# AnnaUshnova/tinyrenderder

Hardware: AMD Instinct MI355X
Metric: triangles/sec (+ Mpixels/sec) at 4096x4096; achieved HBM GB/s vs peak (higher is better)
Workload: dtype f64

## Files before the change

### profiles/binning_bytes.py

```python
import argparse
import csv
import glob
import re
from collections import defaultdict

BIN = ("k_chunk_spine", "k_expand", "k_radix_hist", "k_radix_scan_rows", "k_radix_scatter", "k_bounds", "k_make_items")


def short(name):
    m = re.search(r"k_radix_scatter<(?:\d+, )?(true|false), (true|false)>", name)
    if m:
        return "k_radix_scatter" + (" (last pass)" if m.group(2) == "true" else "")
    for k in BIN + ("k_setup", "k_raster", "k_fold_stats"):
        if k in name:
            return k
    return name.split("(")[0][:38]


ap = argparse.ArgumentParser()
ap.add_argument("--trace")
ap.add_argument("--pmc", nargs="*", default=[])
ap.add_argument("--pairs", type=int, required=True)
ap.add_argument("--tris", type=int, required=True)
ap.add_argument("--old", action="store_true")
a = ap.parse_args()
P, N = a.pairs, a.tris


def binning(name):
    return name.split(" ")[0] in BIN


if a.trace:
    acc = defaultdict(list)
    for f in glob.glob(f"{a.trace}/**/*kernel_trace.csv", recursive=True):
        for r in csv.DictReader(open(f)):
            acc[short(r["Kernel_Name"])].append((int(r["End_Timestamp"]) - int(r["Start_Timestamp"])) / 1e3)
    frames = len(acc["k_setup"])
    print(f"== kernel trace: {frames} frames ==")
    tot = 0.0
    for n, v in sorted(acc.items(), key=lambda kv: -sum(kv[1])):
        tot += sum(v) / frames if binning(n) else 0.0
        print(f"  {n:38s} calls {len(v):4d}  avg {sum(v) / len(v):8.1f} us  median {sorted(v)[len(v) // 2]:8.1f} us  per frame {sum(v) / frames:8.1f} us")
    print(f"  binning kernels per frame: {tot:.1f} us\n")

if a.pmc:
    cnt = defaultdict(lambda: defaultdict(list))
    for d in a.pmc:
        for f in glob.glob(f"{d}/**/*counter_collection.csv", recursive=True):
            per = defaultdict(float)
            for r in csv.DictReader(open(f)):
                n = short(r["Kernel_Name"])
                if binning(n):
                    per[(n, r["Dispatch_Id"], r["Counter_Name"])] += float(r["Counter_Value"])
            for (n, disp, c), v in per.items():
                cnt[n][c].append(v)
    per_frame = {"k_radix_hist": 2, "k_radix_scan_rows": 2, "k_radix_scatter": 2 if a.old else 1}
    if a.old:
        model = {"k_expand": (12 * N, 8 * P), "k_radix_hist": (2 * P, 0), "k_radix_scatter": (8 * P, 8 * P), "k_bounds": (2 * P, 0)}
    else:
        model = {"k_expand": (12 * N, 8 * P), "k_radix_hist": (4 * P, 0), "k_radix_scatter": (8 * P, 8 * P),
                 "k_radix_scatter (last pass)": (8 * P, 6 * P)}
    print("== PMC per dispatch (means) ==")
    for n in sorted(cnt):
        cs = cnt[n]
        print(f"  {n:30s} " + "  ".join(f"{c}={sum(v) / len(v):.4g}" for c, v in sorted(cs.items())))
        act, conf = sum(cs.get("SQ_LDS_IDX_ACTIVE", [0])), sum(cs.get("SQ_LDS_BANK_CONFLICT", [0]))
        if act:
            print(f"  {'':30s} SQ_LDS_BANK_CONFLICT / SQ_LDS_IDX_ACTIVE = {conf / act:.3f}")
    print(f"\n== bytes per frame (P = {P} pairs, N = {N} triangles; MB = 1e6 B) ==")
    print(f"  {'kernel':30s} {'x':>2s} {'read':>8s} {'model':>8s} {'write':>8s} {'model':>8s}")
    tr = tw = mr = mw = 0.0
    for n in sorted(cnt):
        cs = cnt[n]
        if "FETCH_SIZE" not in cs or "WRITE_SIZE" not in cs:
            continue
        k = per_frame.get(n, 1)
        r = 2 * 1024 * sum(cs["FETCH_SIZE"]) / len(cs["FETCH_SIZE"]) * k
        w = 1024 * sum(cs["WRITE_SIZE"]) / len(cs["WRITE_SIZE"]) * k
        m_r, m_w = (x * k for x in model.get(n, (0, 0)))
        tr += r; tw += w; mr += m_r; mw += m_w
        print(f"  {n:30s} {k:2d} {r / 1e6:8.1f} {m_r / 1e6:8.1f} {w / 1e6:8.1f} {m_w / 1e6:8.1f}"
              + (f"   read {100 * (r / m_r - 1):+.0f} %" if m_r else "") + (f", write {100 * (w / m_w - 1):+.0f} %" if m_w else ""))
    print(f"  {'total':30s}    {tr / 1e6:8.1f} {mr / 1e6:8.1f} {tw / 1e6:8.1f} {mw / 1e6:8.1f}")
    print(f"  measured {(tr + tw) / 1e6:.1f} MB against the model's {(mr + mw) / 1e6:.1f} MB: {100 * ((tr + tw) / (mr + mw) - 1):+.1f} %")
```

### tinyrenderder_amd/api.py

```python
from __future__ import annotations

import ctypes as C
import os
import sys

import numpy as np

HERE = os.path.dirname(os.path.abspath(__file__))
LIB_PATH = os.path.join(HERE, "libtrgl.so")

FLAT, GOURAUD, PHONG, EYE, CHECKER = 0, 1, 2, 3, 4
VARY = {FLAT: 0, GOURAUD: 3, PHONG: 24, EYE: 24, CHECKER: 0}
SHADER_USER_FIRST, MAX_USER_SHADERS, MAX_USER_VARY = 64, 32, 64
SHADER_MAY_DISCARD = 1
MAX_USER_VERTEX_SHADERS = 32
MEM_HOST, MEM_DEVICE = 0, 1
PHASE_SETUP, PHASE_BIN, PHASE_RASTER, PHASE_TOTAL, PHASE_RASTER_KERNEL = 0, 1, 2, 3, 4
NUM_PHASES = 5
MAX_TEXTURES = 16
MAX_Z_SNAPSHOTS = 4
MAX_BLUR_RADIUS = 46340
FRUSTUM_LEFT, FRUSTUM_RIGHT, FRUSTUM_BOTTOM, FRUSTUM_TOP, FRUSTUM_NEAR, FRUSTUM_FAR = range(6)

SYMBOLS = [
# ... 31 lines not shown
        return (self.triangles_rasterized, self.fragments_drawn, self.min_x, self.min_y, self.max_x, self.max_y,
                self.min_z, self.max_z, math.copysign(1.0, self.min_z), math.copysign(1.0, self.max_z))


class SsaoParams(C.Structure):
    _fields_ = [("num_directions", C.c_int32), ("steps_per_direction", C.c_int32), ("sample_radius", C.c_double),
                ("occlusion_threshold", C.c_double), ("intensity", C.c_double)]


def make_uniforms(model_view=None, key=(0, 0, 1), fill=(0, 0, 1), rim=(0, 0, 1), normal_map_strength=1.0,
                  tex_diffuse=-1, tex_normal=-1, tex_specular=-1, cells=0) -> Uniforms:
    u = Uniforms()
    mv = np.eye(4) if model_view is None else np.asarray(model_view, np.float64)
    u.model_view[:] = mv.reshape(16).tolist()
    u.key_light_dir_eye[:] = list(map(float, key))
    u.fill_light_dir_eye[:] = list(map(float, fill))
    u.rim_light_dir_eye[:] = list(map(float, rim))
    u.normal_map_strength = float(normal_map_strength)
    u.tex_diffuse, u.tex_normal, u.tex_specular, u.reserved = tex_diffuse, tex_normal, tex_specular, int(cells)
    return u


class TrglError(RuntimeError):
    pass


TRI_REC = np.dtype([(n, "<f8") for n in ("ax", "ay", "s0x", "s0y", "s1x", "s1y", "c0", "uz", "g1", "g2", "ruz", "z0", "z1", "z2")]
                   + [(n, "<u2") for n in ("bx0", "by0", "bx1", "by1")] + [("color", "<u4"), ("dl", "<u4")])
assert TRI_REC.itemsize == 128, "TRI_REC must mirror sizeof(TriRec) == 128"
DBG_RECS, DBG_CNT, DBG_TILEBOX, DBG_VALS, DBG_BMASK, DBG_TILE_START, DBG_TILE_END, DBG_INFO = range(8)
DBG_INFO_FIELDS = ("N", "P", "capacity", "wide", "literal_tris", "large_tris", "zq_cull", "pending", "W", "H", "tiles_x", "tiles_y",
                   "strip_y0", "strip_y1", "strip_ty0", "strip_ty1", "il_tiles", "il_world", "il_rank", "side")
DL_LITERAL = 0x80000000


_lib = None


def load_library(path: str = None):
    global _lib
    if _lib is not None:
        return _lib
    path = path or os.environ.get("TRGL_LIB") or LIB_PATH
    if "torch" not in sys.modules and not os.environ.get("TRGL_NO_TORCH_PRELOAD"):
        try:
            import torch
        except ImportError:
            pass
    if not os.path.exists(path):
        raise TrglError(f"{path} not found: build it with `python -c 'import __graft_entry__ as g; g.build()'` "
                        "(hipcc --offload-arch=gfx950). There is no CPU fallback.")
    L = C.CDLL(path)
    vp, u64p, dp = C.c_void_p, C.POINTER(C.c_uint64), C.POINTER(C.c_double)
    L.trgl_create.argtypes = [C.c_int, C.c_int, C.c_int, C.c_int, C.POINTER(vp)]
    L.trgl_destroy.argtypes = [vp]
    L.trgl_last_error.argtypes = [vp]; L.trgl_last_error.restype = C.c_char_p
    L.trgl_set_viewport.argtypes = [vp, dp]
    L.trgl_init_viewport.argtypes = [vp, C.c_int, C.c_int, C.c_int, C.c_int]
    L.trgl_clear.argtypes = [vp, C.c_void_p, C.c_double]
    L.trgl_upload_texture.argtypes = [vp, C.c_int, C.c_void_p, C.c_int, C.c_int, C.c_int]
    L.trgl_set_strip.argtypes = [vp, C.c_int, C.c_int]
    L.trgl_set_interleave.argtypes = [vp, C.c_int, C.c_int, C.c_int]
    L.trgl_draw.argtypes = [vp, C.c_int, C.POINTER(Uniforms), C.c_void_p, C.c_void_p, C.c_void_p, C.c_uint64, C.c_int]
    L.trgl_flush.argtypes = [vp]
    L.trgl_flush_begin.argtypes = [vp]
    L.trgl_flush_end.argtypes = [vp]
    L.trgl_sync.argtypes = [vp]
    L.trgl_read_framebuffer.argtypes = [vp, C.c_void_p]
    L.trgl_write_framebuffer.argtypes = [vp, C.c_void_p]
    L.trgl_read_zbuffer.argtypes = [vp, C.c_void_p]
    L.trgl_write_zbuffer.argtypes = [vp, C.c_void_p]
    L.trgl_get_stats.argtypes = [vp, C.POINTER(Stats)]
    L.trgl_reset_stats.argtypes = [vp]
    L.trgl_format_stats.argtypes = [C.POINTER(Stats), C.c_char_p, C.c_size_t]
    for name in ("trgl_framebuffer_device_ptr", "trgl_zbuffer_device_ptr", "trgl_stream"):
        getattr(L, name).argtypes = [vp]; getattr(L, name).restype = C.c_void_p
    L.trgl_set_stream.argtypes = [vp, C.c_void_p, C.c_int]
    L.trgl_set_profiling.argtypes = [vp, C.c_int]
    L.trgl_get_phase_ms.argtypes = [vp, dp, u64p]
    L.trgl_reset_phase_ms.argtypes = [vp]
    L.trgl_get_last_flush_info.argtypes = [vp, u64p, u64p, u64p]
    if hasattr(L, "trgl_debug_read"):
        L.trgl_debug_read.argtypes = [vp, C.c_int, C.c_void_p, C.c_size_t, C.POINTER(C.c_size_t)]
    L.trgl_selftest_division.argtypes = [vp, C.c_uint64, C.c_uint64, u64p]
    L.trgl_selftest_sampler.argtypes = [vp, C.c_int, C.c_void_p, C.c_uint64, C.c_void_p]
    L.trgl_draw_indexed.argtypes = [vp, C.c_int, C.POINTER(Uniforms), dp, C.c_void_p, C.c_int, C.c_uint64, C.c_void_p, C.c_uint64, C.c_int]
    L.trgl_ssao_defaults.argtypes = [C.POINTER(SsaoParams)]
    L.trgl_ssao_defaults.restype = None
    L.trgl_postprocess.argtypes = [vp, C.POINTER(SsaoParams), C.c_void_p, C.c_void_p, C.c_void_p]
    L.trgl_obj_load.argtypes = [C.c_char_p, C.POINTER(C.POINTER(C.c_double)), u64p, C.POINTER(C.POINTER(C.c_uint32)), u64p]
    L.trgl_obj_free.argtypes = [C.POINTER(C.c_double), C.POINTER(C.c_uint32)]
    L.trgl_obj_free.restype = None
    L.trgl_tga_max_size.argtypes = [C.c_int, C.c_int, C.c_int]
    L.trgl_tga_max_size.restype = C.c_size_t
    L.trgl_tga_encode.argtypes = [C.c_void_p, C.c_int, C.c_int, C.c_int, C.c_int, C.c_int, C.c_void_p, C.POINTER(C.c_size_t)]
    L.trgl_tga_info.argtypes = [C.c_void_p, C.c_size_t, C.POINTER(C.c_int), C.POINTER(C.c_int), C.POINTER(C.c_int)]
    L.trgl_tga_decode.argtypes = [C.c_void_p, C.c_size_t, C.c_void_p]
    L.trgl_gather.argtypes = [vp, C.c_void_p, C.c_int, C.c_int, C.c_int]
    L.trgl_rccl_unique_id.argtypes = [C.c_void_p]
    L.trgl_rccl_comm_create.argtypes = [C.c_void_p, C.c_int, C.c_int, C.c_int, C.POINTER(C.c_void_p)]
    L.trgl_rccl_comm_destroy.argtypes = [C.c_void_p]
    L.trgl_shader_compile.argtypes = [C.c_char_p, C.c_int, C.c_char_p, C.c_size_t]
    L.trgl_register_shader.argtypes = [vp, C.c_char_p, C.c_int, C.POINTER(C.c_int)]
    L.trgl_shader_compile_ex.argtypes = [C.c_char_p, C.c_int, C.c_uint32, C.c_char_p, C.c_size_t]
    L.trgl_register_shader_ex.argtypes = [vp, C.c_char_p, C.c_int, C.c_uint32, C.POINTER(C.c_int)]
    L.trgl_vertex_shader_compile.argtypes = [C.c_char_p, C.c_int, C.c_char_p, C.c_size_t]
    L.trgl_register_vertex_shader.argtypes = [vp, C.c_char_p, C.c_int, C.POINTER(C.c_int)]
    L.trgl_draw_indexed_vs.argtypes = [vp, C.c_int, C.c_int, C.POINTER(Uniforms), dp, C.c_void_p, C.c_int, C.c_uint64, C.c_void_p, C.c_uint64,
                                       C.c_void_p, C.c_int]
    L.trgl_vertex_stage.argtypes = [vp, C.c_int, C.POINTER(Uniforms), dp, C.c_void_p, C.c_int, C.c_uint64, C.c_void_p, C.c_uint64,
                                    C.c_void_p, C.c_void_p, C.c_int]
    L.trgl_mesh_bounds.argtypes = [vp, C.c_void_p, C.c_int, C.c_uint64, C.c_int, dp, dp]
    for name in ("trgl_mesh_normals", "trgl_mesh_tangents"):
        getattr(L, name).argtypes = [vp, C.c_void_p, C.c_int, C.c_uint64, C.c_void_p, C.c_uint64, C.c_int, C.POINTER(C.c_int)]
    L.trgl_aabb_transform.argtypes = [dp, dp, dp, dp, dp]
    L.trgl_frustum_from_matrix.argtypes = [dp, dp]
    L.trgl_frustum_intersects.argtypes = [dp, dp, dp]
    for name in ("trgl_zbuffer_snapshot", "trgl_zbuffer_restore", "trgl_zbuffer_snapshot_free"):
        getattr(L, name).argtypes = [vp, C.c_int]
    L.trgl_gaussian_kernel.argtypes = [C.c_int, C.c_void_p]
    L.trgl_image_blur.argtypes = [vp, C.c_void_p, C.c_int, C.c_int, C.c_int, C.c_int, C.c_int]
    L.trgl_image_scale.argtypes = [vp, C.c_void_p, C.c_int, C.c_int, C.c_int, C.c_void_p, C.c_int, C.c_int, C.c_int]
    L.trgl_framebuffer_blur.argtypes = [vp, C.c_int]
    for name in SYMBOLS:
        f = getattr(L, name)
        if f.restype is C.c_int and name not in ("trgl_last_error",):
            f.restype = C.c_int
    _lib = L
    return L


def rccl_unique_id() -> bytes:
    L = load_library()
    buf = (C.c_uint8 * 128)()
    rc = L.trgl_rccl_unique_id(buf)
    if rc != 0:
        raise TrglError(f"trgl_rccl_unique_id failed ({rc}): {L.trgl_last_error(None).decode()}")
    return bytes(buf)


def rccl_comm_create(unique_id: bytes, rank: int, world: int, device: int = 0):
    L = load_library()
    comm = C.c_void_p()
    buf = (C.c_uint8 * 128).from_buffer_copy(unique_id)
    rc = L.trgl_rccl_comm_create(buf, rank, world, device, C.byref(comm))
    if rc != 0:
        raise TrglError(f"trgl_rccl_comm_create failed ({rc}): {L.trgl_last_error(None).decode()}")
    return comm


def rccl_comm_destroy(comm):
    load_library().trgl_rccl_comm_destroy(comm)


def shader_compile(source: str, n_varyings: int, may_discard: bool = False):
    L = load_library()
    log = C.create_string_buffer(16384)
    rc = L.trgl_shader_compile_ex(source.encode(), int(n_varyings), SHADER_MAY_DISCARD if may_discard else 0, log, len(log))
    if rc not in (0, -1):
        raise TrglError(f"trgl_shader_compile failed ({rc}): {log.value.decode(errors='replace')}")
    return rc == 0, log.value.decode(errors="replace")


def vertex_shader_compile(source: str, n_varyings: int):
    L = load_library()
    log = C.create_string_buffer(16384)
# ... 526 lines not shown
```

### tinyrenderder_amd/csrc/kernels_bin.hip

```cpp
#include <hip/hip_runtime.h>
#include "trgl_device.h"
#include "launch.h"

namespace {

__device__ __forceinline__ double dmin3(double a, double b, double c) { double m = a; if (b < m) m = b; if (c < m) m = c; return m; }
__device__ __forceinline__ double dmax3(double a, double b, double c) { double m = a; if (m < b) m = b; if (m < c) m = c; return m; }
__device__ __forceinline__ double dot4(const double* m, const double* v) {
    double sum = 0;
    sum += m[0] * v[0]; sum += m[1] * v[1]; sum += m[2] * v[2]; sum += m[3] * v[3];
    return sum;
}

__device__ __forceinline__ int wave_min_i(int v) {
    for (int o = 32; o; o >>= 1) { int t = __shfl_xor(v, o); v = t < v ? t : v; }
    return v;
}
__device__ __forceinline__ int wave_max_i(int v) {
    for (int o = 32; o; o >>= 1) { int t = __shfl_xor(v, o); v = t > v ? t : v; }
    return v;
}

constexpr int SETUP_THREADS = 256;

// ... 161 lines not shown
        if (lit && lane == 0) atomicAdd(&stats->literal_tris, (unsigned long long)__popcll(lit));
        const unsigned long long lrg = __ballot(large);
        if (lrg && lane == 0) atomicAdd(&stats->large_tris, (unsigned long long)__popcll(lrg));
    }
    int wx0 = wave_min_i(bx0), wy0 = wave_min_i(by0), wx1 = wave_max_i(bx1), wy1 = wave_max_i(by1);
    if ((threadIdx.x & 63) == 0 && wx0 != INT_MAX) {
        if (wx0 < __builtin_nontemporal_load(&stats->min_x)) atomicMin(&stats->min_x, wx0);
        if (wy0 < __builtin_nontemporal_load(&stats->min_y)) atomicMin(&stats->min_y, wy0);
        if (wx1 > __builtin_nontemporal_load(&stats->max_x)) atomicMax(&stats->max_x, wx1);
        if (wy1 > __builtin_nontemporal_load(&stats->max_y)) atomicMax(&stats->max_y, wy1);
    }
}

constexpr int SCAN_THREADS = 256;

__device__ __forceinline__ uint32_t wave_incl_scan(uint32_t v) {
    int lane = threadIdx.x & 63;
    for (int o = 1; o < 64; o <<= 1) { uint32_t t = __shfl_up(v, o); if (lane >= o) v += t; }
    return v;
}

__device__ __forceinline__ uint32_t block_excl_scan(uint32_t v, uint32_t* smem , uint32_t* total) {
    uint32_t inc = wave_incl_scan(v);
    int w = threadIdx.x >> 6, lane = threadIdx.x & 63;
    __syncthreads();
    if (lane == 63) smem[w] = inc;
    __syncthreads();
    uint32_t base = 0, tot = 0;
#pragma unroll
    for (int k = 0; k < SCAN_THREADS / 64; ++k) { uint32_t s = smem[k]; if (k < w) base += s; tot += s; }
    *total = tot;
    return base + inc - v;
}

constexpr int EXPAND_CHUNK = 16;

constexpr int SPINE_THREADS = 1024;
__global__ __launch_bounds__(SPINE_THREADS) void k_chunk_spine(const uint32_t* __restrict__ blk_sums, uint32_t nblk,
                                                               uint32_t* __restrict__ chunk_off,
                                                               unsigned long long* __restrict__ total64, unsigned long long* __restrict__ host_copy,
                                                               uint4* __restrict__ bounds16, uint32_t n_half16) {
    __shared__ unsigned long long s_wave[SPINE_THREADS / 64];
    for (uint32_t k = threadIdx.x; k < 2 * n_half16; k += SPINE_THREADS) bounds16[k] = k < n_half16 ? make_uint4(~0u, ~0u, ~0u, ~0u) : make_uint4(0, 0, 0, 0);
    const uint32_t nchunks = (nblk + EXPAND_CHUNK - 1) / EXPAND_CHUNK;
    const int lane = threadIdx.x & 63, w = threadIdx.x >> 6;
    unsigned long long running = 0;
    for (uint32_t start = 0; start < nchunks; start += SPINE_THREADS) {
        const uint32_t c = start + threadIdx.x;
        unsigned long long v = 0;
        if (c < nchunks) {
            const uint32_t q0 = c * EXPAND_CHUNK;
            if (q0 + EXPAND_CHUNK <= nblk) {
                const uint4* p4 = reinterpret_cast<const uint4*>(blk_sums + q0);
#pragma unroll
                for (int k = 0; k < EXPAND_CHUNK / 4; ++k) { const uint4 t = p4[k]; v += (unsigned long long)t.x + t.y + t.z + t.w; }
            } else {
                for (uint32_t q = q0; q < nblk; ++q) v += blk_sums[q];
            }
        }
        unsigned long long inc = v;
        for (int o = 1; o < 64; o <<= 1) { const unsigned long long t = __shfl_up(inc, o); if (lane >= o) inc += t; }
        if (lane == 63) s_wave[w] = inc;
        __syncthreads();
        unsigned long long base = 0, tot = 0;
#pragma unroll
        for (int k = 0; k < SPINE_THREADS / 64; ++k) { const unsigned long long t = s_wave[k]; if (k < w) base += t; tot += t; }
        if (c < nchunks) chunk_off[c] = (uint32_t)(running + base + inc - v);
        running += tot;
        __syncthreads();
    }
    if (threadIdx.x == 0) {
        *total64 = running;
        host_copy[0] = running; host_copy[1] = total64[1]; host_copy[2] = total64[2];
        __threadfence_system();
    }
}

constexpr uint32_t EXPAND_STAGE = 3072;
__device__ __forceinline__ uint32_t tile_block_mask(uint32_t tx, uint32_t ty, uint32_t qx0, uint32_t qy0, uint32_t qx1, uint32_t qy1) {
    const uint32_t c0 = qx0 > 4 * tx ? qx0 - 4 * tx : 0u, c1 = qx1 < 4 * tx + 3 ? qx1 - 4 * tx : 3u;
    const uint32_t r0 = qy0 > 4 * ty ? qy0 - 4 * ty : 0u, r1 = qy1 < 4 * ty + 3 ? qy1 - 4 * ty : 3u;
    return (((2u << c1) - (1u << c0)) & 0xfu) * 0x1111u & ((0xffffu >> (12 - 4 * r1)) & (0xffffu << (4 * r0)));
}
template <bool WIDE>
__global__ __launch_bounds__(256) void k_expand(FrameParams fp, uint32_t first, uint32_t n, int tiles_x, const uint32_t* __restrict__ cnt,
                                                const uint32_t* __restrict__ blk_sums, const uint32_t* __restrict__ chunk_off,
                                                uint32_t blk_base, const uint2* __restrict__ tilebox,
                                                uint32_t* __restrict__ keys, uint32_t* __restrict__ vals, uint16_t* __restrict__ bmask,
                                                const unsigned long long* __restrict__ pairs_total, uint32_t cap) {
    __shared__ uint32_t smem[4];
    __shared__ __attribute__((aligned(16))) uint32_t s_k[EXPAND_STAGE + 4];
    __shared__ __attribute__((aligned(16))) uint32_t s_v[EXPAND_STAGE + 4];
    __shared__ __attribute__((aligned(16))) uint16_t s_m[WIDE ? EXPAND_STAGE + 4 : 4];
    if (*pairs_total > cap) return;
    const uint32_t local = blockIdx.x * blockDim.x + threadIdx.x;
    const uint32_t i = first + local;
    const uint32_t blk = blk_base + blockIdx.x;
    uint32_t c = 0; uint2 tb = make_uint2(0, 0);
    if (local < n) { c = cnt[i]; if (c) tb = tilebox[i]; }
    uint32_t base;
    {
        const uint32_t q0 = blk - blk % EXPAND_CHUNK, l = threadIdx.x & 63u;
        uint32_t part = l < blk - q0 ? blk_sums[q0 + l] : 0u;
        for (int o = 8; o; o >>= 1) part += __shfl_xor(part, o);
        base = chunk_off[blk / EXPAND_CHUNK] + (uint32_t)__builtin_amdgcn_readfirstlane((int)part);
    }
    uint32_t tot;
    const uint32_t o = block_excl_scan(c, smem, &tot);
    const bool staged = tot <= EXPAND_STAGE;
    const uint32_t sh = base & 3u;
    uint32_t* const kdst = keys + base; uint32_t* const vdst = vals + base; uint16_t* const mdst = bmask + base;
    auto put = [&](uint32_t j, uint32_t key, uint32_t iz, uint32_t m) {
        const uint32_t word = WIDE ? key : key | (m << 16);
        if (staged) { s_k[sh + j] = word; s_v[sh + j] = iz; if (WIDE) s_m[sh + j] = (uint16_t)m; }
        else { kdst[j] = word; vdst[j] = iz; if (WIDE) mdst[j] = (uint16_t)m; }
    };
    constexpr uint32_t SMALL = 8;
    if (c && c <= SMALL) {
        const uint32_t qx0 = tb.x & 0x1fff, qy0 = (tb.x >> 16) & 0x1fff, qx1 = tb.y & 0x1fff, qy1 = (tb.y >> 16) & 0x1fff;
        const uint32_t iz = i | ((((tb.x >> 13) & 7u) | (((tb.y >> 13) & 7u) << 3) | ((tb.y >> 29) << 6)) << 25);
        const uint32_t tx0 = qx0 >> 2, ty0 = qy0 >> 2, tx1 = qx1 >> 2;
        uint32_t tx = tx0, row = 0;
        uint32_t ty = fp.il_tiles ? (uint32_t)il_nth_owned_from(fp, (int)ty0, 0) : ty0;
        for (uint32_t k = 0; k < c; ++k) {
            put(o + k, ty * tiles_x + tx, iz, tile_block_mask(tx, ty, qx0, qy0, qx1, qy1));
            if (++tx > tx1) { tx = tx0; ++row; ty = fp.il_tiles ? (uint32_t)il_nth_owned_from(fp, (int)ty0, (int)row) : ty0 + row; }
        }
    }
    unsigned long long big = __ballot(c > SMALL);
    int lane = threadIdx.x & 63;
    while (big) {
        int src = __ffsll((long long)big) - 1;
        big &= big - 1;
        uint32_t cc = __shfl(c, src), oo = __shfl(o, src), ii = __shfl(i, src);
        uint32_t bx = __shfl(tb.x, src), by = __shfl(tb.y, src);
        const uint32_t qx0 = bx & 0x1fff, qy0 = (bx >> 16) & 0x1fff, qx1 = by & 0x1fff, qy1 = (by >> 16) & 0x1fff;
        ii |= (((bx >> 13) & 7u) | (((by >> 13) & 7u) << 3) | ((by >> 29) << 6)) << 25;
        uint32_t tx0 = qx0 >> 2, ty0 = qy0 >> 2, tx1 = qx1 >> 2;
        uint32_t wdt = tx1 - tx0 + 1;
        for (uint32_t k = lane; k < cc; k += 64) {
            uint32_t ty = fp.il_tiles ? (uint32_t)il_nth_owned_from(fp, (int)ty0, (int)(k / wdt)) : ty0 + k / wdt, tx = tx0 + k % wdt;
            put(oo + k, ty * tiles_x + tx, ii, tile_block_mask(tx, ty, qx0, qy0, qx1, qy1));
        }
    }
    if (staged) {
        __syncthreads();
        uint32_t* const kq = keys + (base - sh); uint32_t* const vq = vals + (base - sh); uint16_t* const mq = bmask + (base - sh);
        const uint32_t end = sh + tot;
        for (uint32_t q = threadIdx.x; 4 * q < end; q += 256) {
            const uint32_t j0 = 4 * q;
            if (j0 >= sh && j0 + 4 <= end) {
                *reinterpret_cast<uint4*>(kq + j0) = *reinterpret_cast<const uint4*>(s_k + j0);
                *reinterpret_cast<uint4*>(vq + j0) = *reinterpret_cast<const uint4*>(s_v + j0);
                if (WIDE) *reinterpret_cast<uint2*>(mq + j0) = *reinterpret_cast<const uint2*>(s_m + j0);
            } else {
                for (uint32_t j = j0; j < j0 + 4; ++j)
                    if (j >= sh && j < end) { kq[j] = s_k[j]; vq[j] = s_v[j]; if (WIDE) mq[j] = s_m[j]; }
            }
        }
    }
}

constexpr int RADIX_ROUNDS = 16;
constexpr int RADIX_WAVE_CHUNK = RADIX_ROUNDS * 64;
constexpr uint32_t RADIX_BIG_CAP = 4u << 20;
constexpr int RADIX_MAX_BITS = 8;

__global__ __launch_bounds__(256) void k_radix_hist(const uint32_t* __restrict__ keys, const unsigned long long* __restrict__ pairs_total,
                                                    uint32_t cap, int shift, int bits, uint32_t chunk,
                                                    uint32_t nblocks, uint32_t* __restrict__ hist) {
    __shared__ uint32_t s_cnt[1 << RADIX_MAX_BITS];
    const unsigned long long P64 = *pairs_total;
    const uint32_t P = P64 > cap ? 0u : (uint32_t)P64;
    const uint32_t nb = 1u << bits, mask = nb - 1;
    for (uint32_t b = threadIdx.x; b < nb; b += 256) s_cnt[b] = 0;
    __syncthreads();
    const uint64_t beg = (uint64_t)blockIdx.x * chunk;
    uint64_t end = beg + chunk; if (end > P) end = P;
    for (uint64_t p = beg + 4u * threadIdx.x; p < end; p += 1024) {
        const uint4 q = *reinterpret_cast<const uint4*>(keys + p);
        const uint32_t k[4] = { q.x, q.y, q.z, q.w };
#pragma unroll
        for (int j = 0; j < 4; ++j) if (p + j < end) atomicAdd(&s_cnt[(k[j] >> shift) & mask], 1u);
    }
    __syncthreads();
    for (uint32_t b = threadIdx.x; b < nb; b += 256) hist[(size_t)b * nblocks + blockIdx.x] = s_cnt[b];
}

constexpr int ROWSCAN_THREADS = 1024, ROWSCAN_PER = 8;
__global__ __launch_bounds__(ROWSCAN_THREADS) void k_radix_scan_rows(uint32_t* __restrict__ hist, uint32_t nblocks, uint32_t* __restrict__ totals) {
    __shared__ uint32_t s_wave[ROWSCAN_THREADS / 64];
    uint32_t* row = hist + (size_t)blockIdx.x * nblocks;
    const int lane = threadIdx.x & 63, w = threadIdx.x >> 6;
    uint32_t running = 0;
    for (uint32_t start = 0; start < nblocks; start += ROWSCAN_THREADS * ROWSCAN_PER) {
        const uint32_t base = start + threadIdx.x * ROWSCAN_PER;
        uint32_t v[ROWSCAN_PER], sum = 0;
#pragma unroll
        for (int k = 0; k < ROWSCAN_PER; ++k) { v[k] = (base + k < nblocks) ? row[base + k] : 0; sum += v[k]; }
        uint32_t inc = sum;
        for (int o = 1; o < 64; o <<= 1) { const uint32_t t = __shfl_up(inc, o); if (lane >= o) inc += t; }
        if (lane == 63) s_wave[w] = inc;
        __syncthreads();
        uint32_t wbase = 0, tot = 0;
#pragma unroll
        for (int k = 0; k < ROWSCAN_THREADS / 64; ++k) { const uint32_t t = s_wave[k]; if (k < w) wbase += t; tot += t; }
        uint32_t run = running + wbase + inc - sum;
#pragma unroll
        for (int k = 0; k < ROWSCAN_PER; ++k) { if (base + k < nblocks) row[base + k] = run; run += v[k]; }
        running += tot;
        __syncthreads();
    }
    if (threadIdx.x == 0) totals[blockIdx.x] = running;
}

template <int RADIX_WAVES, bool WIDE, bool LAST>
__global__ __launch_bounds__(RADIX_WAVES * 64) void k_radix_scatter(const uint32_t* __restrict__ keys_in, const uint32_t* __restrict__ vals_in,
                                                                 const uint16_t* __restrict__ msk_in,
                                                                 const unsigned long long* __restrict__ pairs_total, uint32_t cap,
                                                                 int shift, int bits, uint32_t nblocks,
                                                                 const uint32_t* __restrict__ base, const uint32_t* __restrict__ totals,
                                                                 uint32_t* __restrict__ keys_out, uint32_t* __restrict__ vals_out,
                                                                 uint16_t* __restrict__ msk_out,
                                                                 uint32_t* __restrict__ tile_start, uint32_t* __restrict__ tile_end) {
    constexpr int RADIX_THREADS = RADIX_WAVES * 64, RADIX_CHUNK = RADIX_WAVES * RADIX_WAVE_CHUNK;
    __shared__ uint32_t s_cnt[RADIX_WAVES][1 << RADIX_MAX_BITS];
    __shared__ uint32_t s_start[1 << RADIX_MAX_BITS];
    __shared__ uint32_t s_gbase[1 << RADIX_MAX_BITS];
    __shared__ uint32_t s_val[RADIX_CHUNK];
    __shared__ uint32_t s_key[RADIX_CHUNK];
    __shared__ uint16_t s_msk[WIDE ? RADIX_CHUNK : 2];
    const int w = threadIdx.x >> 6, lane = threadIdx.x & 63;
    const unsigned long long P64 = *pairs_total;
    const uint32_t P = P64 > cap ? 0u : (uint32_t)P64;
    if ((uint64_t)blockIdx.x * RADIX_CHUNK >= P) return;
    const uint32_t nb = 1u << bits, mask = nb - 1;
    for (uint32_t b = threadIdx.x; b < nb; b += RADIX_THREADS) {
#pragma unroll
        for (int ww = 0; ww < RADIX_WAVES; ++ww) s_cnt[ww][b] = 0;
        s_gbase[b] = base[(size_t)b * nblocks + blockIdx.x];
    }
    if (w == 0) {
        uint32_t tot[4], run = 0;
#pragma unroll
        for (int q = 0; q < 4; ++q) { const uint32_t d = lane * 4 + q; tot[q] = d < nb ? totals[d] : 0; run += tot[q]; }
        uint32_t inc = run;
        for (int o = 1; o < 64; o <<= 1) { const uint32_t t = __shfl_up(inc, o); if (lane >= o) inc += t; }
        uint32_t ex = inc - run;
#pragma unroll
        for (int q = 0; q < 4; ++q) { const uint32_t d = lane * 4 + q; if (d < nb) s_start[d] = ex; ex += tot[q]; }
    }
    __syncthreads();
    for (uint32_t b = threadIdx.x; b < nb; b += RADIX_THREADS) s_gbase[b] += s_start[b];
    __syncthreads();
    const uint64_t cbeg = (uint64_t)blockIdx.x * RADIX_CHUNK;
    uint64_t cend = cbeg + RADIX_CHUNK; if (cend > P) cend = P;
    const uint32_t n_chunk = (uint32_t)(cend - cbeg);
    const uint64_t wbeg = cbeg + (uint64_t)w * RADIX_WAVE_CHUNK;
    const unsigned long long lt = (1ull << lane) - 1ull;

    uint32_t k[RADIX_ROUNDS], v[RADIX_ROUNDS], rk[RADIX_ROUNDS];
    uint16_t mk[WIDE ? RADIX_ROUNDS : 1];
#pragma unroll
    for (int r = 0; r < RADIX_ROUNDS; ++r) {
        const uint64_t p = wbeg + (uint64_t)r * 64 + lane;
        const bool act = p < cend;
        k[r] = act ? keys_in[p] : 0; v[r] = act ? vals_in[p] : 0;
        if (WIDE) mk[WIDE ? r : 0] = act ? msk_in[p] : (uint16_t)0;
    }
#pragma unroll
    for (int r = 0; r < RADIX_ROUNDS; ++r) {
        const bool act = wbeg + (uint64_t)r * 64 + lane < cend;
        const uint32_t dgt = (k[r] >> shift) & mask;
        unsigned long long same = __ballot(act);
        for (int b = 0; b < bits; ++b) {
            const unsigned long long bal = __ballot((dgt >> b) & 1u);
            same &= ((dgt >> b) & 1u) ? bal : ~bal;
        }
        const uint32_t cur = act ? s_cnt[w][dgt] : 0;
        __builtin_amdgcn_wave_barrier();
        const uint32_t r_in = __popcll(same & lt);
        rk[r] = cur + r_in;
        if (act && r_in == 0) s_cnt[w][dgt] = cur + (uint32_t)__popcll(same);
        __builtin_amdgcn_wave_barrier();
    }
    __syncthreads();
    if (w == 0) {
        uint32_t tot[4], run = 0;
#pragma unroll
        for (int q = 0; q < 4; ++q) {
            const uint32_t d = lane * 4 + q;
            uint32_t t = 0;
            if (d < nb) {
#pragma unroll
                for (int ww = 0; ww < RADIX_WAVES; ++ww) t += s_cnt[ww][d];
            }
            tot[q] = t;
            run += tot[q];
        }
        uint32_t inc = run;
        for (int o = 1; o < 64; o <<= 1) { const uint32_t t = __shfl_up(inc, o); if (lane >= o) inc += t; }
        uint32_t ex = inc - run;
#pragma unroll
        for (int q = 0; q < 4; ++q) { const uint32_t d = lane * 4 + q; if (d < nb) s_start[d] = ex; ex += tot[q]; }
    }
    __syncthreads();
    for (uint32_t d = threadIdx.x; d < nb; d += RADIX_THREADS) {
        uint32_t run = s_start[d];
#pragma unroll
        for (int ww = 0; ww < RADIX_WAVES; ++ww) { const uint32_t c = s_cnt[ww][d]; s_cnt[ww][d] = run; run += c; }
    }
    __syncthreads();
#pragma unroll
    for (int r = 0; r < RADIX_ROUNDS; ++r) {
        if (wbeg + (uint64_t)r * 64 + lane < cend) {
            const uint32_t dgt = (k[r] >> shift) & mask;
            const uint32_t lp = s_cnt[w][dgt] + rk[r];
            s_key[lp] = k[r]; s_val[lp] = v[r];
            if (WIDE) s_msk[lp] = mk[WIDE ? r : 0];
        }
    }
    __syncthreads();
    constexpr uint32_t KEY_MASK = WIDE ? 0xffffffffu : 0xffffu;
    for (uint32_t i = threadIdx.x; i < n_chunk; i += RADIX_THREADS) {
        const uint32_t word = s_key[i];
        const uint32_t dgt = (word >> shift) & mask;
        const uint32_t dst = s_gbase[dgt] + (i - s_start[dgt]);
        vals_out[dst] = s_val[i];
        if (!LAST) {
            keys_out[dst] = word;
            if (WIDE) msk_out[dst] = s_msk[i];
        } else {
            msk_out[dst] = WIDE ? s_msk[i] : (uint16_t)(word >> 16);
            const uint32_t key = word & KEY_MASK;
            if (i == 0 || (s_key[i - 1] & KEY_MASK) != key) atomicMin(&tile_start[key], dst);
            if (i + 1 == n_chunk || (s_key[i + 1] & KEY_MASK) != key) atomicMax(&tile_end[key], dst + 1);
        }
    }
}

}

namespace trgl {

uint32_t setup_num_blocks(uint32_t n) { return (n + SETUP_THREADS - 1) / SETUP_THREADS; }

void launch_setup(hipStream_t s, const FrameParams& fp, const DrawDesc& draw, DrawDesc* draws_dev, int draw_idx, uint32_t n,
                  TriRec* recs, TriW* recs_w, uint32_t* cnt, uint2* tilebox, DevStats* stats, uint32_t* blk_sums, uint32_t blk_base) {
    if (!n) return;
    hipLaunchKernelGGL(k_setup, dim3(setup_num_blocks(n)), dim3(SETUP_THREADS), 0, s, fp, draw, draws_dev, draw_idx, recs, recs_w, cnt, tilebox,
                       stats, blk_sums, blk_base);
}

void launch_chunk_spine(hipStream_t s, const uint32_t* blk_sums, uint32_t nblk, uint32_t* chunk_off, unsigned long long* total64, unsigned long long* host_copy,
                        uint32_t* tile_bounds, size_t half_words) {
    hipLaunchKernelGGL(k_chunk_spine, dim3(1), dim3(SPINE_THREADS), 0, s, blk_sums, nblk, chunk_off, total64, host_copy, (uint4*)tile_bounds,
                       (uint32_t)(half_words / 4));
}

void launch_expand(hipStream_t s, const FrameParams& fp, uint32_t first, uint32_t n, int tiles_x, const uint32_t* cnt, const uint32_t* blk_sums,
                   const uint32_t* chunk_off, uint32_t blk_base, const uint2* tilebox, uint32_t* keys, bool wide, uint32_t* vals, uint16_t* bmask,
                   const unsigned long long* pairs_total, uint32_t cap) {
    if (!n) return;
    if (wide)
        hipLaunchKernelGGL(k_expand<true>, dim3(setup_num_blocks(n)), dim3(SETUP_THREADS), 0, s, fp, first, n, tiles_x, cnt, blk_sums, chunk_off,
                           blk_base, tilebox, keys, vals, bmask, pairs_total, cap);
    else
        hipLaunchKernelGGL(k_expand<false>, dim3(setup_num_blocks(n)), dim3(SETUP_THREADS), 0, s, fp, first, n, tiles_x, cnt, blk_sums, chunk_off,
                           blk_base, tilebox, keys, vals, bmask, pairs_total, cap);
}

static uint32_t radix_waves(uint32_t cap) { return cap >= RADIX_BIG_CAP ? 8u : 4u; }
uint32_t radix_num_workers(uint32_t cap) { const uint64_t chunk = radix_waves(cap) * RADIX_WAVE_CHUNK; return (uint32_t)((cap + chunk - 1) / chunk); }

template <int WAVES, bool WIDE, bool LAST>
static void radix_pass_t(hipStream_t s, const RadixPass& ps, const unsigned long long* pairs_total, uint32_t cap, uint32_t* hist, uint32_t* scan_tmp) {
    const uint32_t nblk = radix_num_workers(cap);
    hipLaunchKernelGGL(k_radix_hist, dim3(nblk), dim3(256), 0, s, ps.keys_in, pairs_total, cap, ps.shift, ps.bits, (uint32_t)(WAVES * RADIX_WAVE_CHUNK),
                       nblk, hist);
    hipLaunchKernelGGL(k_radix_scan_rows, dim3(1u << ps.bits), dim3(ROWSCAN_THREADS), 0, s, hist, nblk, scan_tmp);
    hipLaunchKernelGGL((k_radix_scatter<WAVES, WIDE, LAST>), dim3(nblk), dim3(WAVES * 64), 0, s, ps.keys_in, ps.vals_in, ps.msk_in, pairs_total, cap,
                       ps.shift, ps.bits, nblk, hist, scan_tmp, ps.keys_out, ps.vals_out, ps.msk_out, ps.tile_start, ps.tile_end);
}

template <int WAVES>
static void radix_pass_w(hipStream_t s, const RadixPass& ps, bool wide, bool last, const unsigned long long* pairs_total, uint32_t cap,
                         uint32_t* hist, uint32_t* scan_tmp) {
    if (wide) { if (last) radix_pass_t<WAVES, true, true>(s, ps, pairs_total, cap, hist, scan_tmp); else radix_pass_t<WAVES, true, false>(s, ps, pairs_total, cap, hist, scan_tmp); }
    else { if (last) radix_pass_t<WAVES, false, true>(s, ps, pairs_total, cap, hist, scan_tmp); else radix_pass_t<WAVES, false, false>(s, ps, pairs_total, cap, hist, scan_tmp); }
}

void launch_radix_pass(hipStream_t s, const RadixPass& ps, bool wide, bool last, const unsigned long long* pairs_total, uint32_t cap,
                       uint32_t* hist, uint32_t* scan_tmp) {
    if (!cap) return;
    if (radix_waves(cap) == 8) radix_pass_w<8>(s, ps, wide, last, pairs_total, cap, hist, scan_tmp);
    else radix_pass_w<4>(s, ps, wide, last, pairs_total, cap, hist, scan_tmp);
}

}
```

Measured before the change: 4.112 billion.

## Expand four triangles per thread on big draws; hoist radix scatter loads

k_expand gains a per-thread triangle count template parameter. Draws of at least 393216 triangles process four triangles per thread, using vectorized uint4 loads of counts and tile boxes and one block scan of the per-thread sum, which cuts the scan and launch overhead per triangle. The chunk-offset loads are issued before the overflow check. In the radix scatter kernel, the key, value and mask loads and the base and totals loads are moved ahead of the LDS initialization and digit scan so their latency overlaps that work; out-of-range lanes now load a clamped index instead of branching. A debug override and a crossover profiling script are also added.

```diff
diff --git a/profiles/binning_bytes.py b/profiles/binning_bytes.py
--- a/profiles/binning_bytes.py
+++ b/profiles/binning_bytes.py
@@ -2,6 +2,7 @@
 import csv
 import glob
 import re
+import sqlite3
 from collections import defaultdict
 
 BIN = ("k_chunk_spine", "k_expand", "k_radix_hist", "k_radix_scan_rows", "k_radix_scatter", "k_bounds", "k_make_items")
@@ -23,8 +24,11 @@
 ap.add_argument("--pairs", type=int, required=True)
 ap.add_argument("--tris", type=int, required=True)
 ap.add_argument("--old", action="store_true")
+ap.add_argument("--label", help="printed as a heading above the output (which library the runs are of)")
 a = ap.parse_args()
 P, N = a.pairs, a.tris
+if a.label:
+    print(f"######## {a.label} ########")
 
 
 def binning(name):
@@ -33,9 +37,15 @@
 
 if a.trace:
     acc = defaultdict(list)
-    for f in glob.glob(f"{a.trace}/**/*kernel_trace.csv", recursive=True):
+    traces = glob.glob(f"{a.trace}/**/*kernel_trace.csv", recursive=True)
+    for f in traces:
         for r in csv.DictReader(open(f)):
             acc[short(r["Kernel_Name"])].append((int(r["End_Timestamp"]) - int(r["Start_Timestamp"])) / 1e3)
+    if not traces:
+        q = "select k.display_name, d.start, d.end from rocpd_kernel_dispatch d join rocpd_info_kernel_symbol k on d.kernel_id = k.id"
+        for f in glob.glob(f"{a.trace}/**/*_results.db", recursive=True):
+            for name, t0, t1 in sqlite3.connect(f).execute(q):
+                acc[short(name)].append((t1 - t0) / 1e3)
     frames = len(acc["k_setup"])
     print(f"== kernel trace: {frames} frames ==")
     tot = 0.0
diff --git a/profiles/expand_crossover.py b/profiles/expand_crossover.py
--- /dev/null
+++ b/profiles/expand_crossover.py
@@ -0,0 +1,40 @@
+import csv
+import glob
+import os
+import statistics
+import sys
+
+sys.path.insert(0, os.path.dirname(os.path.dirname(os.path.abspath(__file__))))
+LADDER = (16_384, 65_536, 131_072, 262_144, 393_216, 524_288, 1_048_576, 2_097_152)
+REPS = 9
+
+if "--read" in sys.argv:
+    rows = []
+    for f in glob.glob(f"{sys.argv[sys.argv.index('--read') + 1]}/**/*kernel_trace.csv", recursive=True):
+        rows += [(int(r["Start_Timestamp"]), (int(r["End_Timestamp"]) - int(r["Start_Timestamp"])) / 1e3, r["Kernel_Name"])
+                 for r in csv.DictReader(open(f)) if "k_expand" in r["Kernel_Name"]]
+    rows.sort()
+    assert len(rows) == len(LADDER) * 2 * REPS, len(rows)
+    print("      N   1 a thread   4 a thread   (median us of %d flushes)" % (REPS - 1))
+    for i, n in enumerate(LADDER):
+        t = []
+        for j, per in enumerate((1, 4)):
+            part = rows[(2 * i + j) * REPS:(2 * i + j + 1) * REPS]
+            assert all(f", {per}>" in name for _, _, name in part), part[0][2]
+            t.append(statistics.median(d for _, d, _ in part[1:]))
+        print(f"{n:8d} {t[0]:12.1f} {t[1]:12.1f}")
+else:
+    from tinyrenderder_amd import scenes
+    from tinyrenderder_amd.api import FLAT, Context, load_library
+    L = load_library()
+    W = H = 4096
+    with Context(W, H, 3) as ctx:
+        for n in LADDER:
+            clip, col = scenes.random_triangles(n, W, H, seed=n, rmin=1, rmax=16)
+            for per in (1, 4):
+                assert L.trgl_debug_expand_block(per) == 0
+                for _ in range(REPS):
+                    ctx.clear()
+                    ctx.draw(FLAT, clip, colors=col)
+                    ctx.flush()
+        L.trgl_debug_expand_block(0)
diff --git a/tinyrenderder_amd/api.py b/tinyrenderder_amd/api.py
--- a/tinyrenderder_amd/api.py
+++ b/tinyrenderder_amd/api.py
@@ -137,6 +137,8 @@
     L.trgl_get_last_flush_info.argtypes = [vp, u64p, u64p, u64p]
     if hasattr(L, "trgl_debug_read"):
         L.trgl_debug_read.argtypes = [vp, C.c_int, C.c_void_p, C.c_size_t, C.POINTER(C.c_size_t)]
+    if hasattr(L, "trgl_debug_expand_block"):
+        L.trgl_debug_expand_block.argtypes = [C.c_int]
     L.trgl_selftest_division.argtypes = [vp, C.c_uint64, C.c_uint64, u64p]
     L.trgl_selftest_sampler.argtypes = [vp, C.c_int, C.c_void_p, C.c_uint64, C.c_void_p]
     L.trgl_draw_indexed.argtypes = [vp, C.c_int, C.POINTER(Uniforms), dp, C.c_void_p, C.c_int, C.c_uint64, C.c_void_p, C.c_uint64, C.c_int]
diff --git a/tinyrenderder_amd/csrc/kernels_bin.hip b/tinyrenderder_amd/csrc/kernels_bin.hip
--- a/tinyrenderder_amd/csrc/kernels_bin.hip
+++ b/tinyrenderder_amd/csrc/kernels_bin.hip
@@ -267,7 +267,8 @@
     const uint32_t r0 = qy0 > 4 * ty ? qy0 - 4 * ty : 0u, r1 = qy1 < 4 * ty + 3 ? qy1 - 4 * ty : 3u;
     return (((2u << c1) - (1u << c0)) & 0xfu) * 0x1111u & ((0xffffu >> (12 - 4 * r1)) & (0xffffu << (4 * r0)));
 }
-template <bool WIDE>
+constexpr uint32_t EXPAND_BIG_DRAW = 393216;
+template <bool WIDE, int EXPAND_PER>
 __global__ __launch_bounds__(256) void k_expand(FrameParams fp, uint32_t first, uint32_t n, int tiles_x, const uint32_t* __restrict__ cnt,
                                                 const uint32_t* __restrict__ blk_sums, const uint32_t* __restrict__ chunk_off,
                                                 uint32_t blk_base, const uint2* __restrict__ tilebox,
@@ -277,21 +278,42 @@
     __shared__ __attribute__((aligned(16))) uint32_t s_k[EXPAND_STAGE + 4];
     __shared__ __attribute__((aligned(16))) uint32_t s_v[EXPAND_STAGE + 4];
     __shared__ __attribute__((aligned(16))) uint16_t s_m[WIDE ? EXPAND_STAGE + 4 : 4];
-    if (*pairs_total > cap) return;
-    const uint32_t local = blockIdx.x * blockDim.x + threadIdx.x;
-    const uint32_t i = first + local;
-    const uint32_t blk = blk_base + blockIdx.x;
-    uint32_t c = 0; uint2 tb = make_uint2(0, 0);
-    if (local < n) { c = cnt[i]; if (c) tb = tilebox[i]; }
-    uint32_t base;
-    {
-        const uint32_t q0 = blk - blk % EXPAND_CHUNK, l = threadIdx.x & 63u;
-        uint32_t part = l < blk - q0 ? blk_sums[q0 + l] : 0u;
-        for (int o = 8; o; o >>= 1) part += __shfl_xor(part, o);
-        base = chunk_off[blk / EXPAND_CHUNK] + (uint32_t)__builtin_amdgcn_readfirstlane((int)part);
-    }
+    const unsigned long long P64 = *pairs_total;
+    const uint32_t local0 = (blockIdx.x * blockDim.x + threadIdx.x) * EXPAND_PER;
+    const uint32_t i0 = first + local0;
+    const uint32_t blk = blk_base + blockIdx.x * EXPAND_PER;
+    const uint32_t q0 = blk - blk % EXPAND_CHUNK;
+    uint32_t part = (threadIdx.x & 63u) < blk - q0 ? blk_sums[q0 + (threadIdx.x & 63u)] : 0u;
+    uint32_t base = chunk_off[blk / EXPAND_CHUNK];
+    uint32_t c[EXPAND_PER]; uint2 tb[EXPAND_PER];
+    bool vec = false;
+    if constexpr (EXPAND_PER == 4) vec = (first & 3u) == 0 && local0 + EXPAND_PER <= n;
+    if constexpr (EXPAND_PER == 4) if (vec) {
+        const uint4 cq = *reinterpret_cast<const uint4*>(cnt + i0);
+        const uint4 t01 = *reinterpret_cast<const uint4*>(tilebox + i0), t23 = *reinterpret_cast<const uint4*>(tilebox + i0 + 2);
+        c[0] = cq.x; c[1] = cq.y; c[2] = cq.z; c[3] = cq.w;
+        tb[0] = make_uint2(t01.x, t01.y); tb[1] = make_uint2(t01.z, t01.w); tb[2] = make_uint2(t23.x, t23.y); tb[3] = make_uint2(t23.z, t23.w);
+    }
+    if (!vec) {
+        uint32_t q[EXPAND_PER];
+#pragma unroll
+        for (int j = 0; j < EXPAND_PER; ++j) { q[j] = first + (local0 + j < n ? local0 + j : n - 1); c[j] = cnt[q[j]]; }
+#pragma unroll
+        for (int j = 0; j < EXPAND_PER; ++j) tb[j] = tilebox[q[j]];
+#pragma unroll
+        for (int j = 0; j < EXPAND_PER; ++j) if (local0 + j >= n) c[j] = 0;
+    }
+    if (P64 > cap) return;
+    for (int o = 8; o; o >>= 1) part += __shfl_xor(part, o);
+    base += (uint32_t)__builtin_amdgcn_readfirstlane((int)part);
     uint32_t tot;
-    const uint32_t o = block_excl_scan(c, smem, &tot);
+    uint32_t o[EXPAND_PER];
+    uint32_t csum = 0;
+#pragma unroll
+    for (int j = 0; j < EXPAND_PER; ++j) csum += c[j];
+    o[0] = block_excl_scan(csum, smem, &tot);
+#pragma unroll
+    for (int j = 1; j < EXPAND_PER; ++j) o[j] = o[j - 1] + c[j - 1];
     const bool staged = tot <= EXPAND_STAGE;
     const uint32_t sh = base & 3u;
     uint32_t* const kdst = keys + base; uint32_t* const vdst = vals + base; uint16_t* const mdst = bmask + base;
@@ -301,31 +323,37 @@
         else { kdst[j] = word; vdst[j] = iz; if (WIDE) mdst[j] = (uint16_t)m; }
     };
     constexpr uint32_t SMALL = 8;
-    if (c && c <= SMALL) {
-        const uint32_t qx0 = tb.x & 0x1fff, qy0 = (tb.x >> 16) & 0x1fff, qx1 = tb.y & 0x1fff, qy1 = (tb.y >> 16) & 0x1fff;
-        const uint32_t iz = i | ((((tb.x >> 13) & 7u) | (((tb.y >> 13) & 7u) << 3) | ((tb.y >> 29) << 6)) << 25);
-        const uint32_t tx0 = qx0 >> 2, ty0 = qy0 >> 2, tx1 = qx1 >> 2;
-        uint32_t tx = tx0, row = 0;
-        uint32_t ty = fp.il_tiles ? (uint32_t)il_nth_owned_from(fp, (int)ty0, 0) : ty0;
-        for (uint32_t k = 0; k < c; ++k) {
-            put(o + k, ty * tiles_x + tx, iz, tile_block_mask(tx, ty, qx0, qy0, qx1, qy1));
-            if (++tx > tx1) { tx = tx0; ++row; ty = fp.il_tiles ? (uint32_t)il_nth_owned_from(fp, (int)ty0, (int)row) : ty0 + row; }
-        }
-    }
-    unsigned long long big = __ballot(c > SMALL);
-    int lane = threadIdx.x & 63;
-    while (big) {
-        int src = __ffsll((long long)big) - 1;
-        big &= big - 1;
-        uint32_t cc = __shfl(c, src), oo = __shfl(o, src), ii = __shfl(i, src);
-        uint32_t bx = __shfl(tb.x, src), by = __shfl(tb.y, src);
-        const uint32_t qx0 = bx & 0x1fff, qy0 = (bx >> 16) & 0x1fff, qx1 = by & 0x1fff, qy1 = (by >> 16) & 0x1fff;
-        ii |= (((bx >> 13) & 7u) | (((by >> 13) & 7u) << 3) | ((by >> 29) << 6)) << 25;
-        uint32_t tx0 = qx0 >> 2, ty0 = qy0 >> 2, tx1 = qx1 >> 2;
-        uint32_t wdt = tx1 - tx0 + 1;
-        for (uint32_t k = lane; k < cc; k += 64) {
-            uint32_t ty = fp.il_tiles ? (uint32_t)il_nth_owned_from(fp, (int)ty0, (int)(k / wdt)) : ty0 + k / wdt, tx = tx0 + k % wdt;
-            put(oo + k, ty * tiles_x + tx, ii, tile_block_mask(tx, ty, qx0, qy0, qx1, qy1));
+#pragma unroll
+    for (int j = 0; j < EXPAND_PER; ++j) {
+        if (c[j] && c[j] <= SMALL) {
+            const uint32_t qx0 = tb[j].x & 0x1fff, qy0 = (tb[j].x >> 16) & 0x1fff, qx1 = tb[j].y & 0x1fff, qy1 = (tb[j].y >> 16) & 0x1fff;
+            const uint32_t iz = (i0 + j) | ((((tb[j].x >> 13) & 7u) | (((tb[j].y >> 13) & 7u) << 3) | ((tb[j].y >> 29) << 6)) << 25);
+            const uint32_t tx0 = qx0 >> 2, ty0 = qy0 >> 2, tx1 = qx1 >> 2;
+            uint32_t tx = tx0, row = 0;
+            uint32_t ty = fp.il_tiles ? (uint32_t)il_nth_owned_from(fp, (int)ty0, 0) : ty0;
+            for (uint32_t k = 0; k < c[j]; ++k) {
+                put(o[j] + k, ty * tiles_x + tx, iz, tile_block_mask(tx, ty, qx0, qy0, qx1, qy1));
+                if (++tx > tx1) { tx = tx0; ++row; ty = fp.il_tiles ? (uint32_t)il_nth_owned_from(fp, (int)ty0, (int)row) : ty0 + row; }
+            }
+        }
+    }
+    const int lane = threadIdx.x & 63;
+#pragma unroll
+    for (int j = 0; j < EXPAND_PER; ++j) {
+        unsigned long long big = __ballot(c[j] > SMALL);
+        while (big) {
+            int src = __ffsll((long long)big) - 1;
+            big &= big - 1;
+            uint32_t cc = __shfl(c[j], src), oo = __shfl(o[j], src), ii = __shfl(i0 + j, src);
+            uint32_t bx = __shfl(tb[j].x, src), by = __shfl(tb[j].y, src);
+            const uint32_t qx0 = bx & 0x1fff, qy0 = (bx >> 16) & 0x1fff, qx1 = by & 0x1fff, qy1 = (by >> 16) & 0x1fff;
+            ii |= (((bx >> 13) & 7u) | (((by >> 13) & 7u) << 3) | ((by >> 29) << 6)) << 25;
+            uint32_t tx0 = qx0 >> 2, ty0 = qy0 >> 2, tx1 = qx1 >> 2;
+            uint32_t wdt = tx1 - tx0 + 1;
+            for (uint32_t k = lane; k < cc; k += 64) {
+                uint32_t ty = fp.il_tiles ? (uint32_t)il_nth_owned_from(fp, (int)ty0, (int)(k / wdt)) : ty0 + k / wdt, tx = tx0 + k % wdt;
+                put(oo + k, ty * tiles_x + tx, ii, tile_block_mask(tx, ty, qx0, qy0, qx1, qy1));
+            }
         }
     }
     if (staged) {
@@ -420,39 +448,49 @@
     const uint32_t P = P64 > cap ? 0u : (uint32_t)P64;
     if ((uint64_t)blockIdx.x * RADIX_CHUNK >= P) return;
     const uint32_t nb = 1u << bits, mask = nb - 1;
-    for (uint32_t b = threadIdx.x; b < nb; b += RADIX_THREADS) {
-#pragma unroll
-        for (int ww = 0; ww < RADIX_WAVES; ++ww) s_cnt[ww][b] = 0;
-        s_gbase[b] = base[(size_t)b * nblocks + blockIdx.x];
-    }
-    if (w == 0) {
-        uint32_t tot[4], run = 0;
-#pragma unroll
-        for (int q = 0; q < 4; ++q) { const uint32_t d = lane * 4 + q; tot[q] = d < nb ? totals[d] : 0; run += tot[q]; }
-        uint32_t inc = run;
-        for (int o = 1; o < 64; o <<= 1) { const uint32_t t = __shfl_up(inc, o); if (lane >= o) inc += t; }
-        uint32_t ex = inc - run;
-#pragma unroll
-        for (int q = 0; q < 4; ++q) { const uint32_t d = lane * 4 + q; if (d < nb) s_start[d] = ex; ex += tot[q]; }
-    }
-    __syncthreads();
-    for (uint32_t b = threadIdx.x; b < nb; b += RADIX_THREADS) s_gbase[b] += s_start[b];
-    __syncthreads();
     const uint64_t cbeg = (uint64_t)blockIdx.x * RADIX_CHUNK;
     uint64_t cend = cbeg + RADIX_CHUNK; if (cend > P) cend = P;
     const uint32_t n_chunk = (uint32_t)(cend - cbeg);
     const uint64_t wbeg = cbeg + (uint64_t)w * RADIX_WAVE_CHUNK;
     const unsigned long long lt = (1ull << lane) - 1ull;
 
+    static_assert(RADIX_THREADS >= (1 << RADIX_MAX_BITS), "one digit per thread");
+    const uint32_t col = base[(size_t)(threadIdx.x < nb ? threadIdx.x : mask) * nblocks + blockIdx.x];
+    uint32_t tot[4];
+#pragma unroll
+    for (int q = 0; q < 4; ++q) { const uint32_t d = lane * 4 + q; tot[q] = totals[d < nb ? d : mask]; }
     uint32_t k[RADIX_ROUNDS], v[RADIX_ROUNDS], rk[RADIX_ROUNDS];
     uint16_t mk[WIDE ? RADIX_ROUNDS : 1];
-#pragma unroll
-    for (int r = 0; r < RADIX_ROUNDS; ++r) {
-        const uint64_t p = wbeg + (uint64_t)r * 64 + lane;
-        const bool act = p < cend;
-        k[r] = act ? keys_in[p] : 0; v[r] = act ? vals_in[p] : 0;
-        if (WIDE) mk[WIDE ? r : 0] = act ? msk_in[p] : (uint16_t)0;
-    }
+    {
+        const uint32_t n_wave = wbeg < cend ? (uint32_t)(cend - wbeg < RADIX_WAVE_CHUNK ? cend - wbeg : RADIX_WAVE_CHUNK) : 0u;
+        const uint64_t lbeg = n_wave ? wbeg : cbeg;
+        const uint32_t* const kin = keys_in + lbeg; const uint32_t* const vin = vals_in + lbeg; const uint16_t* const min_ = msk_in + lbeg;
+        const uint32_t li_last = n_wave ? n_wave - 1 : 0u;
+#pragma unroll
+        for (int r = 0; r < RADIX_ROUNDS; ++r) {
+            const uint32_t li = (uint32_t)r * 64 + lane, q = li < n_wave ? li : li_last;
+            k[r] = kin[q]; v[r] = vin[q];
+            if (WIDE) mk[WIDE ? r : 0] = min_[q];
+        }
+    }
+    for (uint32_t b = threadIdx.x; b < nb; b += RADIX_THREADS) {
+#pragma unroll
+        for (int ww = 0; ww < RADIX_WAVES; ++ww) s_cnt[ww][b] = 0;
+    }
+    if (w == 0) {
+        uint32_t run = 0;
+#pragma unroll
+        for (int q = 0; q < 4; ++q) { if (lane * 4 + q >= nb) tot[q] = 0; run += tot[q]; }
+        uint32_t inc = run;
+        for (int o = 1; o < 64; o <<= 1) { const uint32_t t = __shfl_up(inc, o); if (lane >= o) inc += t; }
+        uint32_t ex = inc - run;
+#pragma unroll
+        for (int q = 0; q < 4; ++q) { const uint32_t d = lane * 4 + q; if (d < nb) s_start[d] = ex; ex += tot[q]; }
+    }
+    __syncthreads();
+    if (threadIdx.x < nb) s_gbase[threadIdx.x] = col + s_start[threadIdx.x];
+    __syncthreads();
+
 #pragma unroll
     for (int r = 0; r < RADIX_ROUNDS; ++r) {
         const bool act = wbeg + (uint64_t)r * 64 + lane < cend;
@@ -543,16 +581,18 @@
                        (uint32_t)(half_words / 4));
 }
 
+static int g_expand_per = 0;
 void launch_expand(hipStream_t s, const FrameParams& fp, uint32_t first, uint32_t n, int tiles_x, const uint32_t* cnt, const uint32_t* blk_sums,
                    const uint32_t* chunk_off, uint32_t blk_base, const uint2* tilebox, uint32_t* keys, bool wide, uint32_t* vals, uint16_t* bmask,
                    const unsigned long long* pairs_total, uint32_t cap) {
     if (!n) return;
-    if (wide)
-        hipLaunchKernelGGL(k_expand<true>, dim3(setup_num_blocks(n)), dim3(SETUP_THREADS), 0, s, fp, first, n, tiles_x, cnt, blk_sums, chunk_off,
-                           blk_base, tilebox, keys, vals, bmask, pairs_total, cap);
-    else
-        hipLaunchKernelGGL(k_expand<false>, dim3(setup_num_blocks(n)), dim3(SETUP_THREADS), 0, s, fp, first, n, tiles_x, cnt, blk_sums, chunk_off,
-                           blk_base, tilebox, keys, vals, bmask, pairs_total, cap);
+    const int per = g_expand_per ? g_expand_per : n >= EXPAND_BIG_DRAW ? 4 : 1;
+    const uint32_t nblk = (n + SETUP_THREADS * per - 1) / (SETUP_THREADS * per);
+#define TRGL_EXPAND(W, PER) hipLaunchKernelGGL((k_expand<W, PER>), dim3(nblk), dim3(SETUP_THREADS), 0, s, fp, first, n, tiles_x, cnt, blk_sums, \
+                                               chunk_off, blk_base, tilebox, keys, vals, bmask, pairs_total, cap)
+    if (wide) { if (per == 4) TRGL_EXPAND(true, 4); else TRGL_EXPAND(true, 1); }
+    else { if (per == 4) TRGL_EXPAND(false, 4); else TRGL_EXPAND(false, 1); }
+#undef TRGL_EXPAND
 }
 
 static uint32_t radix_waves(uint32_t cap) { return cap >= RADIX_BIG_CAP ? 8u : 4u; }
@@ -583,3 +623,9 @@
 }
 
 }
+
+extern "C" int trgl_debug_expand_block(int per) {
+    if (per != 0 && per != 1 && per != 4) return 1;
+    trgl::g_expand_per = per;
+    return 0;
+}
```

Result: faster. 4.187 billion, median of 6 (+1.8%).
